# LeCAR-Lab/dial-mpc

Hardware: AMD Instinct MI355X
Metric: sample-rollouts/sec (N x H env.steps), Go2 N=2048 H=16 (higher is better)
Workload: dtype f32

## Files before the change

### dial_mpc_amd/csrc/rollout_body.h

```cpp
#pragma once
#include "derived.h"
#include "dmath.h"

#define MJ_MINVAL 1e-15f
#define MJ_MINIMP 0.0001f
#define MJ_MAXIMP 0.9999f
#define DIAL_PI 3.14159265358979323846f

namespace dial {

template <class D>
inline constexpr bool kNeedL = D::gen;

struct RowRef { int is_lim, dof, c, tan; float f; };
template <class M>
DIAL_DEV int con_of(const M*, const Ws& s, int c) {
  if constexpr (!M::D::gen) return c;
  else return (int)s.clist[c];
}
template <class M>
DIAL_DEV RowRef row_ref(const M* m, const Ws& s, int r) {
  RowRef rr;
  const int nl = dim_nl(m), nlf = nl + dim_nf(m);
  rr.is_lim = r < nlf;
// ... 923 lines not shown
    for (int k = 0; k < 3; k++) { fr[k] = n[k]; fr[3 + k] = bb[k]; fr[6 + k] = cc[k]; }
    float sgn = m->con_kind[c] == DIAL_CON_PLANE_CAPSULE_P ? 1.f : -1.f, hl = m->geom_size[g2][1];
    for (int k = 0; k < 3; k++) ctr[k] += sgn * axis[k] * hl;
  }
  float diff[3] = {ctr[0] - s.gpos[3 * g1], ctr[1] - s.gpos[3 * g1 + 1], ctr[2] - s.gpos[3 * g1 + 2]};
  float dist = dm::dot3(diff, n) - radius;
  s.cdist[c] = dist;
  for (int k = 0; k < 3; k++) s.cpos[3 * c + k] = ctr[k] - n[k] * (radius + 0.5f * dist);
  if constexpr (M::D::ell) s.con_on[c] = (dist - m->con_margin[c]) < 0.f ? 1.f : 0.f;
}

template <class W, class M>
DIAL_DEV void forward_tail(W& w, const M* m, const Ws& s) {
  const int nv = dim_nv(m), nc = dim_nc(m), ne = dim_ne(m), nl = dim_nl(m);
  int nca = nc, nea = ne;
  (void)nv; (void)nl;
  if constexpr (M::D::gen) {
    if (nc <= 64) {
      nca = w.compact(nc, [&](int c) { return s.cdist[c] - m->con_margin[c] < 0.f; }, s.clist);
    } else {
      w.items(nc, [&](int c) { s.clist[c] = (float)c; });
    }
    nea = nl + dim_nf(m) + 4 * nca;
  }
  if constexpr (M::D::gen) {
    if (s.con_cap > 0 && nca > s.con_cap && s.ovf != nullptr) {
      Ws sg = s;
      float* ovf = s.ovf;
#ifndef DIAL_EMU
      asm volatile("" : "+v"(ovf));
#endif
      ws_overflow(sg, ovf, nv, nc, ne);
      forward_constraints(w, m, sg, nca, nea);
      return;
    }
  }
  forward_constraints(w, m, s, nca, nea);
}

template <class W, class M>
DIAL_DEV void forward(W& w, const M* m, const Ws& s) {
  const int nb = dim_nb(m), nv = dim_nv(m), nj = dim_nj(m), ng = dim_ng(m), nsite = dim_ns(m), nc = dim_nc(m);
  const int ne = dim_ne(m), nl = dim_nl(m), ntri = m->ntri;
  int nca = nc, nea = ne;

  if constexpr (W::half2) {
    static_assert(kQuadDims<typename M::D>, "the half-wave kernel exists for the Go2's own instantiation");
    forward_smooth_quad2(w, m, s);
    forward_constraints(w, m, s, nca, nea);
    return;
  } else
  if constexpr (kQuadDims<typename M::D>) {
    forward_smooth_quad(w, m, s);
    forward_constraints(w, m, s, nca, nea);
    return;
  }
  if constexpr (kQuadGenDims<typename M::D>) {
    forward_smooth_quad<false>(w, m, s);
    w.items(nc, [&](int c) { collide_contact(m, s, c); });
    forward_tail(w, m, s);
    return;
  }
  if constexpr (kRowsGenDims<typename M::D>) {
    forward_smooth_rows<true>(w, m, s);
    w.items(nc, [&](int c) { collide_contact(m, s, c); });
    forward_tail(w, m, s);
    return;
  }
  if constexpr (kRowsDims<typename M::D>) {
    forward_smooth_rows(w, m, s);
    {
      DIAL_LANE_SCOPE_IF(DIAL_ROWS_PHASE_SCOPE, w);
      w.items(nc, [&](int c) { collide_contact(m, s, c); });
    }
    forward_constraints(w, m, s, nca, nea);
    return;
  }
  DIAL_MARK(w, 15);
  const bool kin_fast = m->kin_fast != 0;
  if (kin_fast) {
    vfloat L[9];
    w.per_lane_n(L, [&](int b, float* o) {
      for (int k = 0; k < 9; k++) o[k] = 0.f;
      o[7] = -1.f;
      if (b == 0 || b >= nb) return;
      const int bflags = m->body_flags[b];
      float lq[4] = {m->body_quat[b][0], m->body_quat[b][1], m->body_quat[b][2], m->body_quat[b][3]};
      float lp[3] = {m->body_pos[b][0], m->body_pos[b][1], m->body_pos[b][2]};
      if (m->body_jntnum[b] == 1) {
        const int ji = m->body_jntadr[b], qa = m->jnt_qposadr[ji], type = m->jnt_type[ji];
        const float jp[3] = {m->jnt_pos[ji][0], m->jnt_pos[ji][1], m->jnt_pos[ji][2]};
        const float ja[3] = {m->jnt_axis[ji][0], m->jnt_axis[ji][1], m->jnt_axis[ji][2]};
        if (type == DIAL_JNT_FREE) {
          for (int k = 0; k < 3; k++) lp[k] = s.qpos[qa + k];
          for (int k = 0; k < 4; k++) lq[k] = s.qpos[qa + 3 + k];
          dm::normalize4(lq);
          for (int k = 0; k < 4; k++) s.qpos[qa + 3 + k] = lq[k];
        } else if (type == DIAL_JNT_HINGE) {
          float qloc[4], qb[4], t0[3], t1[3];
          dm::axis_angle_to_quat(qloc, ja, s.qpos[qa] - m->qpos0[qa]);
          if (bflags & 1) { qb[0] = qloc[0]; qb[1] = qloc[1]; qb[2] = qloc[2]; qb[3] = qloc[3]; }
          else dm::quat_mul(qb, lq, qloc);
          if (!(bflags & 2)) {
            if (bflags & 1) { t0[0] = jp[0]; t0[1] = jp[1]; t0[2] = jp[2]; }
            else dm::rotate(t0, jp, lq);
            dm::rotate(t1, jp, qb);
// ... 572 lines not shown
  w.items(1 + nq, [&](int it) {
    if (it == 0) s.info[DIAL_INFO_STEP] += 1.f;
    else if (w.out_io && w.out_io->qss) w.out_io->qss[(size_t)w.out_row * nq + (it - 1)] = s.qpos[it - 1];
  });
}

template <bool EPI, class W>
DIAL_DEV int reward_items(const W& w, int n) {
  if constexpr (EPI) return w.epi_cnt;
  else return n;
}

template <bool FULL_INFO, bool PRE = false, bool EPI = false, class W, class M>
DIAL_DEV float env_step(W& w, const M* m, const dial_task* tg, const Ws& s, int st = 0) {
  const int nu = dim_nu(m);
  const bool walk = m->kind == DIAL_TASK_GO2_WALK || m->kind == DIAL_TASK_H1_WALK || m->kind == DIAL_TASK_H1_LOCO ||
                    m->kind == DIAL_TASK_H1_PUSH_CRATE;
  static_assert(!PRE || M::D::pre_ctrl, "control tables: carved for the Dims::pre_ctrl instantiations only");
  if constexpr (PRE) {
    w.jrow = s.jtab + st * nu;
  } else if constexpr (M::D::user_ctrl) {
    w.items(nu, [&](int a) {
      const bool tab = m->table_rows > 0;
      const DialControlIn in = control_in(m, s.info[DIAL_INFO_STEP], s.qpos, s.qvel, s.act, tab ? m->table_ring[m->table_half] : nullptr,
                                          tab ? m->table_cur : 0);
      const float c = dial_user_control(in, a, m->user_params, s.info + DIAL_INFO_USER);
      s.ctrl[a] = c;
      s.info[DIAL_INFO_LAST_CTRL + a] = c;
    });
  } else
  w.items(nu + DIAL_MAX_FEET, [&](int it) {
    if (it < nu) {
      const int a = it;
      const float jt = act2joint(m, s.act[a], a);
      float c;
      if (m->position_control) c = jt;
      else {
        float q_err = jt - s.qpos[7 + a];
        c = dm::clip(m->kp[a] * q_err - m->kd[a] * s.qvel[6 + a], m->tau_range[a][0], m->tau_range[a][1]);
      }
      s.ctrl[a] = c;
    } else {
      const int f = it - nu;
      if (walk && f < m->nfeet) s.ztar[f] = gait_ztar(m, f, s.info[DIAL_INFO_STEP]);
    }
  });
  DIAL_MARK(w, 25);
  const int n_frames = EPI ? 0 : (PRE ? 1 : m->n_frames);
  for (int f = 0; f < n_frames; f++) {
#ifndef DIAL_EMU
    if (w.launder) { asm volatile("" : "+v"(w.lane)); w.lane_r = w.lane; }
#endif
    forward(w, m, s);
    euler(w, m, s);
    DIAL_MARK(w, 9);
  }
  if constexpr (M::D::user) {
    w.items(1, [&](int) {
      float* info = s.info;
      const float step = info[DIAL_INFO_STEP];
      const bool tab = m->table_rows > 0;
      const DialRewardIn in{dim_nq(m), dim_nv(m), nu, dim_nb(m), dim_ns(m), dim_nc(m), step, m->dt,
                            s.qpos, s.qvel, s.xpos, s.xquat, s.spos, s.cdist, s.cpos, s.ctrl, s.act,
                            tab ? m->table_ring[m->table_half] : nullptr, tab ? m->table_cur : 0, m->table, m->table_rows, m->table_cols};
      const float reward = dial_user_reward(in, m->user_params, info + DIAL_INFO_USER);
      if (FULL_INFO) info[DIAL_INFO_DONE] = 0.f;
      info[DIAL_INFO_STEP] = step + 1.f;
      info[DIAL_INFO_REWARD] = reward;
    });
    DIAL_MARK(w, 10);
    return s.info[DIAL_INFO_REWARD];
  }
  if (m->kind == DIAL_TASK_ALLEGRO) {
    w.items(3, [&](int it) {
      const int ob = m->torso_x + 1;
      float acc = 0.f;
      if (it == 0) {
        for (int k = 0; k < 3; k++) { const float e = s.cvel[6 * ob + k] * DIAL_PI / 180.0f - s.info[DIAL_INFO_ANG_VEL_TAR + k]; acc += e * e; }
      } else if (it == 1) {
        for (int k = 0; k < 3; k++) { const float e = s.xpos[3 * ob + k] - s.info[DIAL_INFO_POS_TAR + k]; acc += e * e; }
      } else {
        for (int a = 0; a < nu; a++) { const float e = s.qpos[7 + a] - m->joint_offset[a]; acc += e * e; }
      }
      s.rpart[it] = acc;
    });
    w.items(1, [&](int) {
      const float step = s.info[DIAL_INFO_STEP];
      const float reward = -s.rpart[0] * 1.0f + -s.rpart[1] * 5.0f + -s.rpart[2] * 0.1f;
      if (FULL_INFO) s.info[DIAL_INFO_DONE] = step >= 100.f ? 1.f : 0.f;
      s.info[DIAL_INFO_STEP] = step + 1.f;
      s.info[DIAL_INFO_REWARD] = reward;
    });
    DIAL_MARK(w, 10);
    return s.info[DIAL_INFO_REWARD];
  }
  if constexpr (M::D::gen && ((task_kind_mask<typename M::D>() >> DIAL_TASK_GO2_CRATE) & 1u)) {
    if (m->kind == DIAL_TASK_GO2_CRATE) {
      w.items(1, [&](int) {
        float* info = s.info;
        const int tb = m->torso_x + 1, ub = m->upright_x + 1;
        const float step = info[DIAL_INFO_STEP], dt = m->dt;
        const float tq[4] = {s.xquat[4 * tb], s.xquat[4 * tb + 1], s.xquat[4 * tb + 2], s.xquat[4 * tb + 3]};
        const float uq[4] = {s.xquat[4 * ub], s.xquat[4 * ub + 1], s.xquat[4 * ub + 2], s.xquat[4 * ub + 3]};
        const float hv[3] = {m->head_vec[0], m->head_vec[1], m->head_vec[2]};
        float mat[9], head[3];
        dm::quat_to_mat(mat, tq);
// ... 305 lines not shown
```

### dial_mpc_amd/csrc/rollout_driver.h

```cpp
#pragma once
#include "rollout_body.h"
#include "philox.h"

namespace dial {


template <class W, class M>
DIAL_DEV void load_state(W& w, const M* m, const Ws& s, const float* state) {
  const int nq = dim_nq(m), nv = dim_nv(m);
  DIAL_LANE_SCOPE_IF(M::D::ell, w);
  w.items(nq + 2 * nv + DIAL_INFO_N, [&](int i) {
    float v = state[i];
    if (i < nq) s.qpos[i] = v;
    else if (i < nq + nv) s.qvel[i - nq] = v;
    else if (i < nq + 2 * nv) s.warm[i - nq - nv] = v;
    else s.info[i - nq - 2 * nv] = v;
  });
}
template <class W, class M>
DIAL_DEV void store_state(W& w, const M* m, const Ws& s, float* state) {
  const int nq = dim_nq(m), nv = dim_nv(m);
  DIAL_LANE_SCOPE_IF(M::D::ell, w);
  w.items(nq + 2 * nv + DIAL_INFO_N, [&](int i) {
    float v;
// ... 177 lines not shown
  };
  bool mean_now = false;
  constexpr int KSTRIDE = W::half2 ? 32 : 64, NKEEP = W::half2 ? 4 : 2;
  float keep[NKEEP] = {};
  rsum_t msum = 0;
  (void)packed; (void)keep; (void)msum;
  for (int st_own = st_begin; mean_now || st_own < st_end;) {
    const int st = mean_now ? helper : st_own;
    const int row = mean_now ? io.n_noise : n;
    w.redraw_priority();
#ifndef DIAL_EMU
    if (w.launder) { asm volatile("" : "+v"(w.lane)); w.lane_r = w.lane; }
    if constexpr (M::D::user) {
      if (trows > 0 && !mean_now) {
        const int idx = m->table_nidx, cols = m->table_cols;
        table_publish(w, m, st & 1, idx, cols, tnext);
        if (st + 1 < st_end) {
          M* const c = const_cast<M*>(m);
          const int r = m->table_nr + 1, nidx = table_next_index(idx, r, trows, m->table_mode);
          tnext = table_fetch(m, w.lane, nidx, cols);
          w.sync();
          if (w.lane == 0) { c->table_nidx = nidx; c->table_nr = r; }
        }
      }
    }
#endif
    if constexpr (!PRE) {
      DIAL_LANE_SCOPE_IF(kRowsDims<typename M::D> && !M::D::gen, w);
      w.items(nu, [&](int a) {
        float u;
        if (mean_now && !io.us) {
          u = 0.f;
          for (int k = 0; k < Hn1; k++) u += cfg->W[st][k] * dm::clip(io.Ybar[k * nu + a], -1.f, 1.f);
        } else {
          u = node2u(st, a);
        }
        s.act[a] = u;
      });
    } else {
#ifndef DIAL_EMU
      if (mean_now) {
        w.items(nu, [&](int a) {
          float u = 0.f;
          for (int k = 0; k < Hn1; k++) u += cfg->W[st][k] * dm::clip(io.Ybar[k * nu + a], -1.f, 1.f);
          s.jtab[st * nu + a] = act2joint(m, u, a);
        });
      }
#endif
    }
    DIAL_MARK(w, 11);
    const int work0 = w.work;
    if constexpr (PRE) { w.out_io = &io; w.out_row = row * T + st; }
    if constexpr (W::defer_rewards) reward_rows(w, st);
    float rew = env_step<false, PRE>(w, m, tg, s, st);
    if (mean_now) msum += (rsum_t)rew;
    else if constexpr (!W::defer_rewards) rsum += (rsum_t)rew;
#ifndef DIAL_EMU
    if constexpr (M::D::ell) {
      if (io.work_stat && relay < 0) {
        int lvl = 0;
        if (w.lane == 0) {
          const int tot_w = atomicAdd(io.work_stat, w.work - work0) + (w.work - work0);
          const int tot_s = atomicAdd(io.work_stat + 1, 1) + 1;
          const float own = (float)w.work * (float)tot_s, avg = (float)tot_w * (float)(st + 1 - st_begin);
#ifndef DIAL_LAG_T1
#define DIAL_LAG_T1 1.0f
#define DIAL_LAG_T2 1.2f
#define DIAL_LAG_T3 1.4f
#endif
          lvl = own > DIAL_LAG_T3 * avg ? 3 : (own > DIAL_LAG_T2 * avg ? 2 : (own > DIAL_LAG_T1 * avg ? 1 : 0));
        }
        w.prio_level = __builtin_amdgcn_readfirstlane(lvl);
      }
    }
#endif
    const size_t o = (size_t)row * T + st;
    if constexpr (!PRE) {
      float* const qrow = io.qss ? io.qss + o * nq : nullptr;
      float* const qdrow = io.qdss ? io.qdss + o * nv : nullptr;
      float* const xrow = io.xss ? io.xss + o * nx : nullptr;
      float* const rrow = io.rewss ? io.rewss + o : nullptr;
      const int nmax = nx > nq ? nx : nq;
      w.items(nmax, [&](int i) {
        if (qrow && i < nq) qrow[i] = s.qpos[i];
        if (qdrow && i < nv) qdrow[i] = s.qvel[i];
        if (xrow && i < nx) xrow[i] = s.xpos[3 + i];
        if (rrow && i == 0) rrow[0] = rew;
      });
    }
    (void)o;
#ifndef DIAL_PROFILE
    if constexpr (TRACE) { if (io.trace) store_state(w, m, s, io.trace + o * nstate); }
#endif
    DIAL_MARK(w, 24);
#ifndef DIAL_EMU
    if (mean_now) {
      if (helper + 1 < T) {
        store_state(w, m, s, io.relay_buf);
        w.items(1, [&](int) { store_sum(io.relay_buf + nstate, msum); });
        __builtin_amdgcn_fence(__ATOMIC_RELEASE, "agent");
        if (w.lane == 0) __hip_atomic_store(io.relay_flag, helper + 1, __ATOMIC_RELEASE, __HIP_MEMORY_SCOPE_AGENT);
      } else {
        if (io.rews) { const float mean = (float)(msum / (rsum_t)T); w.items(1, [&](int) { io.rews[row] = mean; }); }
        if (w.lane == 0) __hip_atomic_store(io.relay_flag, 0, __ATOMIC_RELEASE, __HIP_MEMORY_SCOPE_AGENT);
      }
      w.items(KSTRIDE, [&](int l) {
// ... 122 lines not shown
```

### dial_mpc_amd/csrc/solver_reg.h

```cpp
#pragma once

namespace dial {

template <int N> constexpr int kCholStride = (N + 3) & ~3;

template <class Topo, int N>
struct ElimOrder {
  int seq[N > 0 ? N : 1] = {};
  int nlevel = 0;
  int lvl[N > 0 ? N + 1 : 2] = {};
  constexpr ElimOrder() {
    int depth[N > 0 ? N : 1] = {};
    int maxd = 0;
    for (int i = 0; i < N; i++) {
      int d = 0;
      for (int j = 0; j < i; j++) d += Topo::anc(i, j) ? 1 : 0;
      depth[i] = d;
      maxd = d > maxd ? d : maxd;
    }
    int t = 0;
    for (int d = maxd; d >= 0; d--) {
      lvl[nlevel++] = t;
      for (int i = N - 1; i >= 0; i--)
        if (depth[i] == d) seq[t++] = N - 1 - i;
// ... 138 lines not shown
    w.dup_rows(b, bX, bY);
    static_for<l0, l1>([&](auto STEP) {
      constexpr int kp = EO.seq[STEP];
      const vfloat col = a[kp];
      vfloat cX, cY;
      w.dup_rows(col, cX, cY);
      const vfloat rinv = w.template rcp_pick<kp>(cX, cY);
      const vfloat lik = vsel(w.lane_gt(kp), col * rinv, vsplat(0.f));
      a[kp] = lik;
      dinv = vsel(w.lane_eq(kp), rinv, dinv);
      constexpr AncList<Topo, N, kp> L{};
      static_for<0, L.n>([&](auto IDX) {
        constexpr int jp = L.jp[IDX];
        a[jp] = w.template fnma_pick<jp>(a[jp], cX, cY, lik);
      });
    });
    static_for<l0, l1>([&](auto STEP) { constexpr int kp = EO.seq[STEP]; b = w.template fnma_pick<kp>(b, bX, bY, a[kp]); });
  });
  w.items(N, [&](int l) {
    static_for<0, N>([&](auto KP) { constexpr int kp = KP; scratch[(N - 1 - kp) * S + own_i(l)] = lane_val(a[kp], l); });
  });
  if (dinv_io) *dinv_io = dinv;
  }
  vfloat x = b * dinv;
  static_for<0, S / 4>([&](auto Q) {
    constexpr int q = Q;
    vfloat t[4];
    w.per_lane4([&](int l) { return scratch + (l < N ? own_i(l) : 0) * S + 4 * q; }, t[0], t[1], t[2], t[3]);
    static_for<0, 4>([&](auto E) {
      constexpr int j = 4 * q + E;
      if constexpr (j < N) a[N - 1 - j] = t[E];
    });
  });
  static_for<0, EO.nlevel>([&](auto LVR) {
    constexpr int lv = EO.nlevel - 1 - LVR, l0 = EO.lvl[lv], l1 = EO.lvl[lv + 1];
    vfloat xX, xY;
    w.dup_rows(x, xX, xY);
    static_for<l0, l1>([&](auto STEP) { constexpr int kp = EO.seq[STEP]; x = w.template fnma_pick<kp>(x, xX, xY, a[kp]); });
  });
  return w.lane_reverse(x, N);
}


#ifndef DIAL_CHOL_DPP
#define DIAL_CHOL_DPP 1
#endif
template <class D, class TopoT = typename D::Topo, bool REUSE = false, class W, class M>
DIAL_DEV vfloat reg_chol(W& w, const M* m, const float* A, vfloat bvec, float* scratch, vfloat* dinv_io = nullptr) {
  constexpr bool go2_one = std::is_same<D, DimsGo2>::value && !W::half2;
  if constexpr (W::half2 || (DIAL_CHOL_DPP && !go2_one)) return reg_chol_solve2<D, TopoT, REUSE>(w, m, A, bvec, scratch, dinv_io);
  else return reg_chol_solve_v<D, TopoT, REUSE>(w, m, A, bvec, scratch, dinv_io);
}

template <class W, class M>
DIAL_DEV void solver_reg(W& w, const M* m, const Ws& s) {
  constexpr int NV = M::D::NV, NC = M::D::NC, NL = M::D::NL;
  constexpr int C0 = 32;
  static_assert(NV <= 32 && 4 * NC <= 32, "lane layout needs nv <= 32 and 4*ncon <= 32");
  w.begin_region();
  const vbool isdof = w.lane_lt(NV);
  const vfloat vzero = vsplat(0.f);

  auto row_of = [&](int l) -> int {
    if (l < NV) return m->dof_limrow[l];
    if (l >= C0 && l < C0 + 4 * NC) return NL + (l - C0);
    return -1;
  };
  vfloat R[NV];
  {
    constexpr int S = M::D::S, T = M::D::T;
    const auto fetch = [&](int l, int j) {
      const int ojc = (int)(s.Jc - s.M), ozero = (int)(s.lsign - s.M) + NL;
      const int off = l < NV ? l * S : ((l >= C0 && l < C0 + 4 * NC) ? ojc + (l - C0) : ozero);
      const int stride = l < NV ? 1 : ((l >= C0 && l < C0 + 4 * NC) ? T : 0);
      return s.M[off + j * stride];
    };
#pragma unroll
    for (int j = 0; j < NV; j++) {
      if constexpr (NV > 20) R[j] = w.per_lane_r([&](int l) { return fetch(l, j); });
      else R[j] = w.per_lane([&](int l) { return fetch(l, j); });
    }
  }
  const vfloat vD = w.per_lane([&](int l) { int r = row_of(l); return r >= 0 ? s.D[r] : 0.f; });
  const vfloat varef = w.per_lane([&](int l) { int r = row_of(l); return r >= 0 ? s.aref[r] : 0.f; });
  const vfloat vls = w.per_lane([&](int l) { int r = l < NV ? m->dof_limrow[l] : -1; return r >= 0 ? s.lsign[r] : 0.f; });
  const vfloat vqfs = w.per_lane([&](int l) { return l < NV ? s.qfs[l] : 0.f; });
  const vfloat vqas = w.per_lane([&](int l) { return l < NV ? s.qas[l] : 0.f; });
  const vfloat vwarm = w.per_lane([&](int l) { return l < NV ? s.warm[l] : 0.f; });

#ifndef DIAL_SWEEP_DPP
#define DIAL_SWEEP_DPP 1
#endif
  auto dotR = [&](const vfloat& v) {
    vfloat acc[3] = {vzero, vzero, vzero};
#if DIAL_SWEEP_DPP
    vfloat vlo, vhi, X, Y;
    w.dup_halves(v, vlo, vhi);
    w.dup_rows(vlo, X, Y);
    static_for<0, NV>([&](auto IDX) { constexpr int j = IDX; acc[j % 3] = w.template fma_pick<j>(acc[j % 3], X, Y, R[j]); });
#else
    float sb[3] = {0.f, 0.f, 0.f};
    static_for<0, NV + 2>([&](auto IDX) {
      constexpr int idx = IDX;
      if constexpr (idx < NV) sb[idx % 3] = bcast(v, idx);
      if constexpr (idx >= 2) acc[(idx - 2) % 3] = acc[(idx - 2) % 3] + R[idx - 2] * sb[(idx - 2) % 3];
    });
#endif
    return (acc[0] + acc[1]) + acc[2];
  };
  auto row_prod = [&](const vfloat& v, const vfloat& sweep) { return vsel(isdof, vls * v, sweep); };
  auto row_cost_terms = [&](const vfloat& ja) { return vsel(vlt0(ja), vD * ja * ja, vzero); };

  const vfloat pW = dotR(vwarm), pS = dotR(vqas);
  const vfloat jaW = row_prod(vwarm, pW) - varef, jaS = row_prod(vqas, pS) - varef;
  const vfloat maW = vsel(isdof, pW, vzero), maS = vsel(isdof, pS, vzero);
  float cw, gw, cs, gs;
  {
    vfloat t[4] = {row_cost_terms(jaW), (maW - vqfs) * (vwarm - vqas), row_cost_terms(jaS), (maS - vqfs) * (vqas - vqas)};
    float r[4];
    w.vsumN(t, r);
    cw = r[0]; gw = r[1]; cs = r[2]; gs = r[3];
  }
  const float cost_w = 0.5f * cw + 0.5f * gw, cost_s = 0.5f * cs + 0.5f * gs;
  const bool use_warm = cost_w < cost_s;
  vfloat vqacc = use_warm ? vwarm : vqas;
  vfloat vMa = use_warm ? maW : maS;
  vfloat vJa = use_warm ? jaW : jaS;
  float cost = use_warm ? cost_w : cost_s;
  float gauss = use_warm ? 0.5f * gw : 0.5f * gs;
  float prev_cost = INFINITY;
  const float scale = 1.f / (m->meaninertia * (float)(NV > 1 ? NV : 1));
  const bool rule_swap = m->ls_rule == DIAL_LS_SWAP;
  const int max_iter = DM_UNIFORM_I(m->iterations), max_ls = DM_UNIFORM_I(m->ls_iterations);
  const float tol = m->tolerance, ls_tol = m->ls_tolerance, meaninertia = m->meaninertia;

#ifdef DIAL_PROFILE
  unsigned long long prof_prev_act = 0;
#endif
  int niter = 0;
  unsigned long long act_prev = 0;
  vfloat h_dinv = vzero;
  bool h_valid = false;
  for (;;) {
    const vbool act = vlt0(vJa);
#ifdef DIAL_PROFILE
    {
      const unsigned long long cur = __builtin_amdgcn_ballot_w64(act && (vD > 0.f));
      static_assert(sizeof(cur) == 8, "");
      if (niter == 1 && w.lane == 0 && w.acc) { w.acc[28] += 1; if (cur == prof_prev_act) w.acc[29] += 1; }
      prof_prev_act = cur;
    }
#endif
    const vfloat vf = vsel(act, vD * (vzero - vJa), vzero);
    vfloat qfc = vls * vf;
#if DIAL_SWEEP_DPP
    vfloat flo, fhi, fX, fY;
    w.dup_halves(vf, flo, fhi);
    w.dup_rows(fhi, fX, fY);
#endif
    static_for<0, NC>([&](auto Cc) {
      constexpr int c = Cc;
      vfloat jr[4];
      w.per_lane4([&](int l) { return s.Jc + (l < NV ? l : 0) * M::D::T + 4 * c; }, jr[0], jr[1], jr[2], jr[3]);
#if DIAL_SWEEP_DPP
      const vfloat t01 = w.template fma_pick<4 * c + 1>(w.template mul_pick<4 * c>(fX, fY, jr[0]), fX, fY, jr[1]);
      const vfloat t23 = w.template fma_pick<4 * c + 3>(w.template mul_pick<4 * c + 2>(fX, fY, jr[2]), fX, fY, jr[3]);
      qfc = qfc + (t01 + t23);
#else
      qfc = qfc + ((jr[0] * bcast(vf, C0 + 4 * c) + jr[1] * bcast(vf, C0 + 4 * c + 1)) +
                   (jr[2] * bcast(vf, C0 + 4 * c + 2) + jr[3] * bcast(vf, C0 + 4 * c + 3)));
#endif
    });
    const vfloat vgrad = vsel(isdof, vMa - vqfs - qfc, vzero);
    float gn = 0.f;
    if (niter > 0) {
      vfloat t[3] = {row_cost_terms(vJa), (vMa - vqfs) * (vqacc - vqas), vgrad * vgrad};
      float r[3];
      w.vsumN(t, r);
      gauss = 0.5f * r[1];
      prev_cost = cost;
      cost = 0.5f * r[0] + gauss;
      gn = r[2];
    } else if (max_iter != 1) {
      gn = w.vsum(vgrad * vgrad);
    }
    DIAL_MARK(w, 4);
    bool done;
    if (max_iter != 1) {
      const float improvement = scale * (prev_cost - cost), gradient = scale * DM_SQRT(gn);
      done = niter >= max_iter || improvement < tol || gradient < tol;
    } else {
      done = niter >= 1;
    }
    if (done) break;

    const vfloat vwgt = vsel(act, vD, vzero);
#ifdef DIAL_NO_FACTOR_REUSE
    const bool reuse = false;
#else
    const unsigned long long act_now = w.mask(vlt0(vzero - vwgt));
    const bool reuse = h_valid && act_now == act_prev;
    act_prev = act_now;
    h_valid = true;
#endif
    vfloat vsearch;
    if (reuse) {
      vsearch = vzero - reg_chol<typename M::D, typename M::D::Topo, true>(w, m, s.H, vgrad, s.H, &h_dinv);
      DIAL_MARK(w, 5);
    } else {
    {
      constexpr int S = M::D::S, T = M::D::T, NLP = M::D::NLP, NP = M::D::NHI / 64;
      (void)S;
      w.items(64, [&](int l) {
        const int r = row_of(l);
        if (r >= 0) s.frc[r < NL ? r : NLP + (r - NL)] = lane_val(vwgt, l);
        if (l == 63) s.frc[NLP + 4 * NC] = 0.f;
      });
      vfloat part[NP], tot[NP];
      static_for<0, 4>([&](auto Qq) {
        constexpr int q = Qq;
        bool any = false;
        static_for<0, NP>([&](auto PASS) { any = any || q < m->hpass_n[PASS]; });
        if (any) {
          vfloat ji[NP][4], jj[NP][4], dd[NP][4];
          static_for<0, NP>([&](auto PASS) {
            constexpr int pass = PASS;
            const auto c4 = [&](int l) { return (int)((m->hrec[pass * 64 + l][0] >> (20 + 3 * q)) & 7u) * 4; };
            w.per_lane4([&](int l) { return s.Jc + (m->hrec[pass * 64 + l][0] & 1023u) + c4(l); }, ji[pass][0], ji[pass][1], ji[pass][2], ji[pass][3]);
            w.per_lane4([&](int l) { return s.Jc + ((m->hrec[pass * 64 + l][0] >> 10) & 1023u) + c4(l); }, jj[pass][0], jj[pass][1], jj[pass][2], jj[pass][3]);
            w.per_lane4([&](int l) { return s.frc + NLP + c4(l); }, dd[pass][0], dd[pass][1], dd[pass][2], dd[pass][3]);
          });
          static_for<0, NP>([&](auto PASS) {
            constexpr int pass = PASS;
            const vfloat t = ((ji[pass][0] * dd[pass][0]) * jj[pass][0] + (ji[pass][1] * dd[pass][1]) * jj[pass][1]) +
                             ((ji[pass][2] * dd[pass][2]) * jj[pass][2] + (ji[pass][3] * dd[pass][3]) * jj[pass][3]);
            const vfloat tq = w.per_lane([&](int l) { return q < (int)(m->hrec[pass * 64 + l][1] >> 29) ? lane_val(t, l) : 0.f; });
            if constexpr (q == 0) part[pass] = tq; else part[pass] = part[pass] + tq;
          });
        }
      });
      static_for<0, NP>([&](auto PASS) {
        constexpr int pass = PASS;
        const vfloat pair = part[pass] + w.quad_xor1(part[pass]);
        const vfloat quad = pair + w.quad_xor2(pair);
        tot[pass] = w.per_lane([&](int l) {
          const float t1 = lane_val(part[pass], l), t2 = lane_val(pair, l), t4 = lane_val(quad, l);
          const uint32_t pc = (m->hrec[pass * 64 + l][1] >> 26) & 3u;
// ... 44 lines not shown
      ljv[q] = w.per_lane([&](int l) { const int r = (l & 15) + 16 * q; return (l < 48 && r < NE) ? s.jv[r] : 0.f; });
      const vfloat lD = w.per_lane([&](int l) { const int r = (l & 15) + 16 * q; return (l < 48 && r < NE) ? s.D[r] : 0.f; });
      const vfloat dja = lD * lJa[q], djv = lD * ljv[q];
      Q0[q] = (lJa[q] * 0.5f) * dja;
      Q1[q] = ljv[q] * dja;
      Q2[q] = (ljv[q] * 0.5f) * djv;
    }
    vfloat pk[4];
    auto ls_eval3 = [&](float a0, float a1, float a2) {
      const vfloat va = vsel(g0, vsplat(a0), vsel(g01, vsplat(a1), vsplat(a2)));
      vfloat s0 = vzero, s1v = vzero, s2v = vzero;
#pragma unroll
      for (int q = 0; q < RPL; q++) {
        const vfloat act = vsel(vlt0(lJa[q] + ljv[q] * va), vsplat(1.f), vzero);
        s0 = s0 + act * Q0[q];
        s1v = s1v + act * Q1[q];
        s2v = s2v + act * Q2[q];
      }
      w.row16_sum3(s0, s1v, s2v);
      const vfloat q0 = s0 + vsplat(qg0), q1 = s1v + vsplat(qg1), q2 = s2v + vsplat(qg2);
      const vfloat vcost = (va * va) * q2 + va * q1 + q0;
      const vfloat vd0 = vfma(va * 2.f, q2, q1);
      const vfloat vd1 = q2 * 2.f + vsel(veq0(q2), vsplat(MJ_MINVAL), vzero);
      w.per_lane_n(pk, [&](int l, float* o) {
        ls_pack(lane_val(va, l), lane_val(vcost, l), lane_val(vd0, l), lane_val(vd1, l), o[0], o[1], o[2], o[3]);
      });
    };
    auto point_at = [&](int lane) {
      LsPt p;
      p.alpha = fbits(bcast(pk[0], lane)); p.nalpha = fbits(bcast(pk[1], lane)); p.cost = fbits(bcast(pk[2], lane)); p.d0 = fbits(bcast(pk[3], lane));
      return p;
    };
    ls_eval3(0.f, 0.f, 0.f);
    const LsPt p0 = point_at(0);
    ls_eval3(bitsf(p0.nalpha), bitsf(p0.nalpha), bitsf(p0.nalpha));
    LsPt lo, hi;
    ls_open(p0, point_at(0), lo, hi);
    const int kg = DM_UNIFORM_I(fkey(gtol)), kng = DM_UNIFORM_I(fkey(-gtol));
    const LsGate gate = ls_gate(kg, kng);
    int ls_iter = 0;
    while (ls_iter < max_ls) {
      DM_NOFOLD();
      if (ls_converged_lo(lo, gate)) break;
      DM_NOFOLD();
      if (ls_converged_hi(hi, gate)) break;
      ls_eval3(bitsf(lo.nalpha), bitsf(hi.nalpha), 0.5f * (bitsf(lo.alpha) + bitsf(hi.alpha)));
      const bool swap = ls_update_lazy(rule_swap, lo, hi, fbits(bcast(pk[3], 0)), fbits(bcast(pk[3], 16)), fbits(bcast(pk[3], 32)), 0, 16, 32,
                                       [&](int word, int lane) { return fbits(bcast(pk[word], lane)); });
      ls_iter++;
      if (!swap) break;
    }
    float alpha;
    const bool improved = ls_result(p0, lo, hi, alpha);
    if (improved) {
      vqacc = vqacc + vsearch * alpha;
      vMa = vMa + vmv * alpha;
      vJa = vJa + vjv * alpha;
    }
    niter++;
#ifdef DIAL_PROFILE
    if (w.lane == 0 && w.acc) { w.acc[30] += ls_iter; w.acc[31] += 1; }
#endif
    DIAL_MARK(w, 7);
  }
  w.items(NV, [&](int i) {
    const float q = lane_val(vqacc, i);
    s.qacc[i] = q;
    s.warm[i] = q;
  });
  DIAL_MARK(w, 8);
}

}
```

### dial_mpc_amd/csrc/wave.h

```cpp
#pragma once
#include "rollout_io.h"

#ifdef DIAL_EMU
#include <cmath>
#include <cstdio>
#include <cstring>
#include <vector>
#define DIAL_DEV inline
#define DIAL_UNROLL


struct vbool { bool x[64]; };
struct vfloat {
  float x[64];
};
inline vfloat vsplat(float v) { vfloat r; for (int l = 0; l < 64; l++) r.x[l] = v; return r; }
inline vfloat operator+(const vfloat& a, const vfloat& b) { vfloat r; for (int l = 0; l < 64; l++) r.x[l] = a.x[l] + b.x[l]; return r; }
inline vfloat operator-(const vfloat& a, const vfloat& b) { vfloat r; for (int l = 0; l < 64; l++) r.x[l] = a.x[l] - b.x[l]; return r; }
inline vfloat operator*(const vfloat& a, const vfloat& b) { vfloat r; for (int l = 0; l < 64; l++) r.x[l] = a.x[l] * b.x[l]; return r; }
inline vfloat operator*(const vfloat& a, float b) { vfloat r; for (int l = 0; l < 64; l++) r.x[l] = a.x[l] * b; return r; }
inline vfloat vfma(const vfloat& a, const vfloat& b, const vfloat& c) { vfloat r; for (int l = 0; l < 64; l++) r.x[l] = std::fma(a.x[l], b.x[l], c.x[l]); return r; }
inline vfloat vsel(const vbool& c, const vfloat& a, const vfloat& b) { vfloat r; for (int l = 0; l < 64; l++) r.x[l] = c.x[l] ? a.x[l] : b.x[l]; return r; }
inline vbool vlt0(const vfloat& a) { vbool r; for (int l = 0; l < 64; l++) r.x[l] = a.x[l] < 0.f; return r; }
inline vbool veq0(const vfloat& a) { vbool r; for (int l = 0; l < 64; l++) r.x[l] = a.x[l] == 0.f; return r; }
inline float bcast(const vfloat& v, int lane) { return v.x[lane]; }
inline float lane_val(const vfloat& v, int lane) { return v.x[lane]; }
inline void load2(const float* p, float& a, float& b) { a = p[0]; b = p[1]; }
inline void load4(const float* p, float& a, float& b, float& c, float& d) { a = p[0]; b = p[1]; c = p[2]; d = p[3]; }
inline void store2(float* p, float a, float b) { p[0] = a; p[1] = b; }
inline void store4(float* p, float a, float b, float c, float d) { p[0] = a; p[1] = b; p[2] = c; p[3] = d; }
inline float fast_rsqrt(float x) { return 1.0f / std::sqrt(x); }
inline float fast_rcp(float x) { return 1.0f / x; }
inline vfloat vrcp(const vfloat& a) { vfloat r; for (int l = 0; l < 64; l++) r.x[l] = 1.0f / a.x[l]; return r; }

inline float emu_row_tree(const float* v) {
  float s1[16], s2[16], s3[16];
  for (int l = 0; l < 16; l++) s1[l] = v[l] + v[l ^ 1];
  for (int l = 0; l < 16; l++) s2[l] = s1[l] + s1[l ^ 2];
  for (int l = 0; l < 16; l++) s3[l] = s2[l] + s2[(l & 8) | (7 - (l & 7))];
  return s3[15] + s3[0];
}
inline float emu_tree64(const float* v) {
  const float r0 = emu_row_tree(v), r1 = emu_row_tree(v + 16), r2 = emu_row_tree(v + 32), r3 = emu_row_tree(v + 48);
  return (r3 + r2) + (r1 + r0);
}
inline float emu_tree32(const float* v) {
  return emu_row_tree(v) + emu_row_tree(v + 16);
}

#define DIAL_MARK(w, id)
#define DIAL_LANE_SCOPE(w)
#define DIAL_LANE_SCOPE_IF(cond, w)
struct Wave {
  static constexpr bool half2 = false;
  static constexpr bool defer_rewards = false;
  bool tree_sums = false;
  bool launder = false;
  const dial::RolloutIO* out_io = nullptr;
  int out_row = 0;
  const float* jrow = nullptr;
  float* lds = nullptr;
  int lds_words = 0;
  bool check_races = false;
  int races = 0;
  int phase = 0;

  bool nancheck = false, nan_seen = false;
  void scan_nonfinite() {
    if (!nancheck || nan_seen) return;
    for (int k = 0; k < lds_words; k++)
      if (!std::isfinite(lds[k])) {
        std::fprintf(stderr, "[wave_emu] first non-finite LDS word after phase #%d: word %d = %g\n", phase, k, (double)lds[k]);
        nan_seen = true;
        return;
      }
  }
  template <class F>
  void items(int count, F f) {
    phase++;
    if (!check_races) {
      for (int i = 0; i < count; i++) f(i);
      scan_nonfinite();
      return;
    }
    std::vector<float> snap(lds, lds + lds_words);
    for (int i = 0; i < count; i++) f(i);
    std::vector<float> fwd(lds, lds + lds_words);
    std::memcpy(lds, snap.data(), sizeof(float) * lds_words);
    for (int i = count - 1; i >= 0; i--) f(i);
    if (std::memcmp(fwd.data(), lds, sizeof(float) * lds_words) != 0) {
      if (races < 10) {
        int w = 0;
        for (; w < lds_words; w++)
          if (std::memcmp(&fwd[w], &lds[w], 4) != 0) break;
        std::fprintf(stderr, "[wave_emu] intra-phase dependence in phase #%d (first differing LDS word %d)\n", phase, w);
      }
      races++;
    }
  }
  template <class F>
  float sum(int count, F f) {
    if (tree_sums) {
      float v[64];
      for (int l = 0; l < 64; l++) { v[l] = l < count ? f(l) : 0.f; for (int i = l + 64; i < count; i += 64) v[l] += f(i); }
      return emu_tree64(v);
    }
    float s = 0.f;
    for (int i = 0; i < count; i++) s += f(i);
// ... 66 lines not shown
      float t = 0.f;
      for (int l = 0; l < 16; l++) t += v.x[16 * g + l];
      for (int l = 0; l < 16; l++) r.x[16 * g + l] = t;
    }
    return r;
  }
  void row16_sum3(vfloat& a, vfloat& b, vfloat& c) { a = row16_sum(a); b = row16_sum(b); c = row16_sum(c); }
  template <class F>
  int compact(int count, F pred, float* list) {
    int n = 0;
    for (int l = 0; l < count && l < 64; l++) if (pred(l)) list[n++] = (float)l;
    return n;
  }
  template <int K>
  void row16_sumN(vfloat (&v)[K]) { for (int k = 0; k < K; k++) v[k] = row16_sum(v[k]); }
  template <int K>
  void seg8_sumN(vfloat (&v)[K]) {
    for (int k = 0; k < K; k++) {
      vfloat s1, s2, s3;
      for (int l = 0; l < 64; l++) s1.x[l] = v[k].x[l] + v[k].x[l ^ 1];
      for (int l = 0; l < 64; l++) s2.x[l] = s1.x[l] + s1.x[l ^ 2];
      for (int l = 0; l < 64; l++) s3.x[l] = s2.x[l] + s2.x[(l & ~7) | (7 - (l & 7))];
      v[k] = s3;
    }
  }
  template <class F>
  vfloat gather64(const vfloat& v, F src) { vfloat r; for (int l = 0; l < 64; l++) r.x[l] = v.x[src(l) & 63]; return r; }
  float vsum(const vfloat& v) { if (tree_sums) return emu_tree64(v.x); float s = 0.f; for (int l = 0; l < 64; l++) s += v.x[l]; return s; }
  template <int K>
  void vsumN(vfloat (&v)[K], float (&out)[K]) { for (int k = 0; k < K; k++) out[k] = vsum(v[k]); }
  template <int K>
  float bc(const vfloat& v) { return v.x[K]; }
  void dup_rows(const vfloat& v, vfloat& X, vfloat& Y) {
    for (int l = 0; l < 64; l++) { X.x[l] = v.x[(l & 32) | (l & 15)]; Y.x[l] = v.x[(l & 32) | 16 | (l & 15)]; }
  }
  void dup_halves(const vfloat& v, vfloat& LO, vfloat& HI) {
    for (int l = 0; l < 64; l++) { LO.x[l] = v.x[l & 31]; HI.x[l] = v.x[32 | (l & 31)]; }
  }
  template <int K>
  float rowbc(const vfloat& v) { return v.x[K]; }
  template <int K>
  vfloat mul_pick(const vfloat& X, const vfloat& Y, const vfloat& other) { return other * pick<K>(X, Y); }
  template <int K>
  vfloat pick(const vfloat& X, const vfloat& Y) { if constexpr (K < 16) return row_bcast<K>(X); else return row_bcast<K - 16>(Y); }
  template <int K>
  vfloat fma_pick(const vfloat& acc, const vfloat& X, const vfloat& Y, const vfloat& other) { return acc + other * pick<K>(X, Y); }
  template <int K>
  vfloat fnma_pick(const vfloat& acc, const vfloat& X, const vfloat& Y, const vfloat& other) { return acc - other * pick<K>(X, Y); }
  template <int K>
  vfloat rcp_pick(const vfloat& X, const vfloat& Y) { return vrcp(pick<K>(X, Y)); }
};
struct WaveD : Wave {
  static constexpr bool defer_rewards = true;
  float* stash = nullptr;
  float* srow = nullptr;
  float* zrow = nullptr;
  float* zbase = nullptr;
  int epi_cnt = 0;
};

struct WaveH : Wave {
  static constexpr bool half2 = true;
  template <class F>
  float sum(int count, F f) {
    float v[32];
    for (int l = 0; l < 32; l++) { v[l] = l < count ? f(l) : 0.f; for (int i = l + 32; i < count; i += 32) v[l] += f(i); }
    return emu_tree32(v);
  }
  template <class F>
  void sum3(int count, F f, float& a, float& b, float& c) {
    float va[32], vb[32], vc[32];
    for (int l = 0; l < 32; l++) {
      va[l] = vb[l] = vc[l] = 0.f;
      if (l < count) f(l, va[l], vb[l], vc[l]);
      for (int i = l + 32; i < count; i += 32) { float x = 0.f, y = 0.f, z = 0.f; f(i, x, y, z); va[l] += x; vb[l] += y; vc[l] += z; }
    }
    a = emu_tree32(va); b = emu_tree32(vb); c = emu_tree32(vc);
  }
  template <class F>
  vfloat per_lane(F f) { vfloat r; for (int l = 0; l < 64; l++) r.x[l] = f(l & 31); return r; }
  template <class F>
  vfloat per_lane_r(F f) { return per_lane(f); }
  template <int K, class F>
  void per_lane_n(vfloat (&out)[K], F f) {
    for (int l = 0; l < 64; l++) { float o[K]; f(l & 31, o); for (int k = 0; k < K; k++) out[k].x[l] = o[k]; }
  }
  template <class F>
  void per_lane4(F f, vfloat& a, vfloat& b, vfloat& c, vfloat& d) {
    for (int l = 0; l < 64; l++) { const float* p = f(l & 31); a.x[l] = p[0]; b.x[l] = p[1]; c.x[l] = p[2]; d.x[l] = p[3]; }
  }
  unsigned long long mask(const vbool& c) const { unsigned long long b = 0; for (int l = 0; l < 32; l++) b |= (unsigned long long)(c.x[l] ? 1 : 0) << l; return b; }
  vbool lane_gt(int k) const { vbool r; for (int l = 0; l < 64; l++) r.x[l] = (l & 31) > k; return r; }
  vbool lane_eq(int k) const { vbool r; for (int l = 0; l < 64; l++) r.x[l] = (l & 31) == k; return r; }
  vbool lane_lt(int k) const { vbool r; for (int l = 0; l < 64; l++) r.x[l] = (l & 31) < k; return r; }
  vfloat lane_reverse(const vfloat& v, int n) { vfloat r; for (int l = 0; l < 64; l++) r.x[l] = (l & 31) < n ? v.x[(l & 32) + n - 1 - (l & 31)] : 0.f; return r; }
  float vsum(const vfloat& v) { return emu_tree32(v.x); }
  template <int K>
  void vsumN(vfloat (&v)[K], float (&out)[K]) { for (int k = 0; k < K; k++) out[k] = vsum(v[k]); }
  template <class F>
  vfloat gather(const vfloat& v, F src) { vfloat r; for (int l = 0; l < 64; l++) r.x[l] = v.x[(l & 32) | (src(l & 31) & 31)]; return r; }
  vfloat grp8_bcast3(const vfloat& v) { vfloat r; for (int l = 0; l < 64; l++) r.x[l] = v.x[(l & ~7) | 3]; return r; }
};

#else
#include <hip/hip_runtime.h>
#define DIAL_DEV __device__ __forceinline__
// ... 31 lines not shown

using vfloat = float;
using vbool = bool;
__device__ __forceinline__ vfloat vsplat(float v) { return v; }
__device__ __forceinline__ vfloat vfma(vfloat a, vfloat b, vfloat c) { return __builtin_fmaf(a, b, c); }
__device__ __forceinline__ vfloat vsel(vbool c, vfloat a, vfloat b) { return c ? a : b; }
__device__ __forceinline__ vbool vlt0(vfloat a) { return a < 0.f; }
__device__ __forceinline__ vbool veq0(vfloat a) { return a == 0.f; }
__device__ __forceinline__ float bcast(vfloat v, int lane) {
  return __builtin_bit_cast(float, __builtin_amdgcn_readlane(__builtin_bit_cast(int, v), lane));
}
__device__ __forceinline__ float lane_val(vfloat v, int) { return v; }
__device__ __forceinline__ void load2(const float* p, float& a, float& b) { const float2 t = *reinterpret_cast<const float2*>(p); a = t.x; b = t.y; }
__device__ __forceinline__ void load4(const float* p, float& a, float& b, float& c, float& d) { const float4 t = *reinterpret_cast<const float4*>(p); a = t.x; b = t.y; c = t.z; d = t.w; }
__device__ __forceinline__ void store2(float* p, float a, float b) { *reinterpret_cast<float2*>(p) = make_float2(a, b); }
__device__ __forceinline__ void store4(float* p, float a, float b, float c, float d) { *reinterpret_cast<float4*>(p) = make_float4(a, b, c, d); }
__device__ __forceinline__ float fast_rsqrt(float x) { return __builtin_amdgcn_rsqf(x); }
__device__ __forceinline__ float fast_rcp(float x) { return __builtin_amdgcn_rcpf(x); }
__device__ __forceinline__ vfloat vrcp(vfloat a) { return __builtin_amdgcn_rcpf(a); }

template <class W>
struct LaneScope {
  W& w;
  int keep, keep_r;
  __device__ __forceinline__ explicit LaneScope(W& w_) : w(w_), keep(w_.lane), keep_r(w_.lane_r) {
    int lq = w.lane;
    asm volatile("" : "+v"(lq));
    w.lane = lq;
    w.lane_r = lq;
  }
  __device__ __forceinline__ ~LaneScope() { w.lane = keep; w.lane_r = keep_r; }
};
#define DIAL_LANE_SCOPE(w) LaneScope<std::remove_reference_t<decltype(w)>> dial_lane_scope_(w)
template <bool COND, class W>
struct LaneScopeIf {
  __device__ __forceinline__ explicit LaneScopeIf(W&) {}
};
template <class W>
struct LaneScopeIf<true, W> : LaneScope<W> {
  __device__ __forceinline__ explicit LaneScopeIf(W& w_) : LaneScope<W>(w_) {}
};
#define DIAL_LANE_SCOPE_IF(cond, w) LaneScopeIf<(cond), std::remove_reference_t<decltype(w)>> dial_lane_scope_if_(w)
#ifdef DIAL_PROFILE
#define DIAL_NSEC 32
#define DIAL_MARK(w, id) (w).mark(id)
#elif defined(DIAL_ISA_MARKS)
#define DIAL_MARK(w, id) asm volatile("; DIAL_MARK %0" ::"n"(id))
#else
#define DIAL_MARK(w, id)
#endif
struct Wave {
  static constexpr bool half2 = false;
  static constexpr bool defer_rewards = false;
  int lane;
  const dial::RolloutIO* out_io = nullptr;
  int out_row = 0;
  const float* jrow = nullptr;
#ifdef DIAL_PROFILE
  unsigned long long tprev = 0;
  unsigned long long* acc = nullptr;
  __device__ __forceinline__ void mark(int id) {
    unsigned long long t = __builtin_readcyclecounter();
    if (lane == 0 && acc) acc[id] += t - tprev;
    tprev = t;
  }
#endif
  __device__ __forceinline__ void sync() {
#ifdef DIAL_BLOCK_SYNC
    __syncthreads();
#else
    __builtin_amdgcn_fence(__ATOMIC_RELEASE, "wavefront");
    __builtin_amdgcn_wave_barrier();
    __builtin_amdgcn_fence(__ATOMIC_ACQUIRE, "wavefront");
#endif
  }

  template <class F>
  __device__ __forceinline__ void items(int count, F f) {
    for (int i = lane; i < count; i += 64) f(i);
    sync();
  }
  template <class F>
  __device__ __forceinline__ float sum(int count, F f) {
    float v = lane < count ? f(lane) : 0.f;
    for (int i = lane + 64; i < count; i += 64) v += f(i);
    return dialwave::wave_sum(v);
  }
  template <class F>
  __device__ __forceinline__ void sum3(int count, F f, float& a, float& b, float& c) {
    float x = 0.f, y = 0.f, z = 0.f;
    if (lane < count) f(lane, x, y, z);
    for (int i = lane + 64; i < count; i += 64) {
      float x2 = 0.f, y2 = 0.f, z2 = 0.f;
      f(i, x2, y2, z2);
      x += x2; y += y2; z += z2;
    }
    vfloat t3[3] = {x, y, z};
    float r3[3];
    vsumN(t3, r3);
    a = r3[0]; b = r3[1]; c = r3[2];
  }
  template <class F>
  __device__ __forceinline__ float maxv(int count, F f) {
    float v = lane < count ? f(lane) : -INFINITY;
    for (int i = lane + 64; i < count; i += 64) { const float u = f(i); v = u > v ? u : v; }
    return dialwave::wave_max_shfl(v);
// ... 152 lines not shown
    Y = __builtin_bit_cast(float, r1);
#ifdef DIAL_FUSED_DPP
    asm("s_nop 1" : "+v"(X), "+v"(Y));
#endif
  }
  __device__ __forceinline__ void dup_halves(vfloat v, vfloat& LO, vfloat& HI) {
    const auto r = __builtin_amdgcn_permlane32_swap(__builtin_bit_cast(unsigned, v), __builtin_bit_cast(unsigned, v), false, false);
    const unsigned r0 = r[0], r1 = r[1];
    LO = __builtin_bit_cast(float, r0);
    HI = __builtin_bit_cast(float, r1);
  }
  template <int K>
  __device__ __forceinline__ float rowbc(vfloat v) { return row_bcast<K>(v); }
  template <int K>
  __device__ __forceinline__ vfloat pick(vfloat X, vfloat Y) { if constexpr (K < 16) return row_bcast<K>(X); else return row_bcast<K - 16>(Y); }
#ifdef DIAL_FUSED_DPP
#define DIAL_DPP_TAIL " row_newbcast:%3 row_mask:0xf bank_mask:0xf bound_ctrl:1"
  template <int K>
  __device__ __forceinline__ vfloat fma_pick(vfloat acc, vfloat X, vfloat Y, vfloat other) {
    asm("v_fmac_f32_dpp %0, %1, %2" DIAL_DPP_TAIL : "+v"(acc) : "v"(K < 16 ? X : Y), "v"(other), "n"(K & 15));
    return acc;
  }
  template <int K>
  __device__ __forceinline__ vfloat fnma_pick(vfloat acc, vfloat X, vfloat Y, vfloat other) {
    asm("v_fmac_f32_dpp %0, -%1, %2" DIAL_DPP_TAIL : "+v"(acc) : "v"(K < 16 ? X : Y), "v"(other), "n"(K & 15));
    return acc;
  }
  template <int K>
  __device__ __forceinline__ vfloat rcp_pick(vfloat X, vfloat Y) {
    vfloat r;
    asm("v_rcp_f32_dpp %0, %1 row_newbcast:%2 row_mask:0xf bank_mask:0xf bound_ctrl:1" : "=v"(r) : "v"(K < 16 ? X : Y), "n"(K & 15));
    return r;
  }
  template <int K>
  __device__ __forceinline__ vfloat mul_pick(vfloat X, vfloat Y, vfloat other) {
    vfloat r;
    asm("v_mul_f32_dpp %0, %1, %2" DIAL_DPP_TAIL : "=v"(r) : "v"(K < 16 ? X : Y), "v"(other), "n"(K & 15));
    return r;
  }
#undef DIAL_DPP_TAIL
#else
  template <int K>
  __device__ __forceinline__ vfloat mul_pick(vfloat X, vfloat Y, vfloat other) { return other * pick<K>(X, Y); }
  template <int K>
  __device__ __forceinline__ vfloat fma_pick(vfloat acc, vfloat X, vfloat Y, vfloat other) { return acc + other * pick<K>(X, Y); }
  template <int K>
  __device__ __forceinline__ vfloat fnma_pick(vfloat acc, vfloat X, vfloat Y, vfloat other) { return acc - other * pick<K>(X, Y); }
  template <int K>
  __device__ __forceinline__ vfloat rcp_pick(vfloat X, vfloat Y) { return vrcp(pick<K>(X, Y)); }
#endif
};
struct WaveD : Wave {
  static constexpr bool defer_rewards = true;
  float* stash = nullptr;
  float* srow = nullptr;
  float* zrow = nullptr;
  float* zbase = nullptr;
  int epi_cnt = 0;
};

struct WaveH : Wave {
  static constexpr bool half2 = true;
  int half;
  __device__ __forceinline__ void init(int tid) { lane = tid & 31; lane_r = lane; half = (tid >> 5) & 1; }
  template <class F>
  __device__ __forceinline__ void items(int count, F f) {
    for (int i = lane; i < count; i += 32) f(i);
    sync();
  }
  static __device__ __forceinline__ float half_combine(float v) {
    const auto r = __builtin_amdgcn_permlane16_swap(__builtin_bit_cast(unsigned, v), __builtin_bit_cast(unsigned, v), false, false);
    const unsigned r0 = r[0], r1 = r[1];
    return __builtin_bit_cast(float, r0) + __builtin_bit_cast(float, r1);
  }
  template <int K>
  __device__ __forceinline__ float bc(vfloat v) {
    static_assert(K >= 0 && K < 32, "logical lane");
    vfloat X, Y;
    dup_rows(v, X, Y);
    if constexpr (K < 16) return row_bcast<K>(X);
    else return row_bcast<K - 16>(Y);
  }
  template <class F>
  __device__ __forceinline__ vfloat gather(vfloat v, F src) { return __shfl(v, (src(lane) & 31) + 32 * half, 64); }
  __device__ __forceinline__ vfloat grp8_bcast3(vfloat v) {
    const vfloat a = row_bcast<3>(v), b = row_bcast<11>(v);
    return (lane & 8) ? b : a;
  }

  static __device__ __forceinline__ float opaque(float v) { asm("" : "+v"(v)); return v; }
  __device__ __forceinline__ vfloat row16_sum(vfloat v) { return Wave::row16_sum(opaque(v)); }
  template <int K>
  __device__ __forceinline__ void row16_sumN(vfloat (&v)[K]) {
#pragma unroll
    for (int k = 0; k < K; k++) v[k] = opaque(v[k]);
    Wave::row16_sumN(v);
  }
  __device__ __forceinline__ void row16_sum3(vfloat& a, vfloat& b, vfloat& c) { a = opaque(a); b = opaque(b); c = opaque(c); Wave::row16_sum3(a, b, c); }
  __device__ __forceinline__ float vsum(vfloat v) { return half_combine(row16_sum(v)); }
  template <int K>
  __device__ __forceinline__ void vsumN(vfloat (&v)[K], float (&out)[K]) {
    row16_sumN(v);
#pragma unroll
    for (int k = 0; k < K; k++) out[k] = half_combine(v[k]);
  }
  template <class F>
// ... 49 lines not shown
```

Baseline: 6.032 million.

## Skip dead final-step work and trim last solver iteration in deferred-reward waves

```diff
diff --git a/dial_mpc_amd/csrc/rollout_body.h b/dial_mpc_amd/csrc/rollout_body.h
--- a/dial_mpc_amd/csrc/rollout_body.h
+++ b/dial_mpc_amd/csrc/rollout_body.h
@@ -999,6 +999,7 @@
   } else
   if constexpr (kQuadDims<typename M::D>) {
     forward_smooth_quad(w, m, s);
+    if constexpr (W::lean_tail_cut) { if (w.tail_cut) return; }
     forward_constraints(w, m, s, nca, nea);
     return;
   }
@@ -1677,6 +1678,9 @@
     if (w.launder) { asm volatile("" : "+v"(w.lane)); w.lane_r = w.lane; }
 #endif
     forward(w, m, s);
+    if constexpr (W::lean_tail_cut) {
+      if (w.tail_cut) { DIAL_MARK(w, 9); return 0.f; }
+    }
     euler(w, m, s);
     DIAL_MARK(w, 9);
   }
diff --git a/dial_mpc_amd/csrc/rollout_driver.h b/dial_mpc_amd/csrc/rollout_driver.h
--- a/dial_mpc_amd/csrc/rollout_driver.h
+++ b/dial_mpc_amd/csrc/rollout_driver.h
@@ -253,6 +253,7 @@
     const int work0 = w.work;
     if constexpr (PRE) { w.out_io = &io; w.out_row = row * T + st; }
     if constexpr (W::defer_rewards) reward_rows(w, st);
+    if constexpr (W::lean_tail_cut) w.tail_cut = (st + 1 == T && !io.qss && !io.qdss && helper < 0 && !mean_now) ? 1 : 0;
     float rew = env_step<false, PRE>(w, m, tg, s, st);
     if (mean_now) msum += (rsum_t)rew;
     else if constexpr (!W::defer_rewards) rsum += (rsum_t)rew;
diff --git a/dial_mpc_amd/csrc/solver_reg.h b/dial_mpc_amd/csrc/solver_reg.h
--- a/dial_mpc_amd/csrc/solver_reg.h
+++ b/dial_mpc_amd/csrc/solver_reg.h
@@ -214,6 +214,9 @@
   else return reg_chol_solve_v<D, TopoT, REUSE>(w, m, A, bvec, scratch, dinv_io);
 }
 
+#ifndef DIAL_SOLVER_EXIT_HOOK
+#define DIAL_SOLVER_EXIT_HOOK(at_cap)
+#endif
 template <class W, class M>
 DIAL_DEV void solver_reg(W& w, const M* m, const Ws& s) {
   constexpr int NV = M::D::NV, NC = M::D::NC, NL = M::D::NL;
@@ -303,15 +306,18 @@
   unsigned long long act_prev = 0;
   vfloat h_dinv = vzero;
   bool h_valid = false;
+#ifdef DIAL_PROFILE
+  const auto prof_active_set = [&](const vfloat& ja) {
+    const unsigned long long cur = __builtin_amdgcn_ballot_w64(vlt0(ja) && (vD > 0.f));
+    static_assert(sizeof(cur) == 8, "");
+    if (niter == 1 && w.lane == 0 && w.acc) { w.acc[28] += 1; if (cur == prof_prev_act) w.acc[29] += 1; }
+    prof_prev_act = cur;
+  };
+#endif
   for (;;) {
     const vbool act = vlt0(vJa);
 #ifdef DIAL_PROFILE
-    {
-      const unsigned long long cur = __builtin_amdgcn_ballot_w64(act && (vD > 0.f));
-      static_assert(sizeof(cur) == 8, "");
-      if (niter == 1 && w.lane == 0 && w.acc) { w.acc[28] += 1; if (cur == prof_prev_act) w.acc[29] += 1; }
-      prof_prev_act = cur;
-    }
+    prof_active_set(vJa);
 #endif
     const vfloat vf = vsel(act, vD * (vzero - vJa), vzero);
     vfloat qfc = vls * vf;
@@ -354,7 +360,7 @@
     } else {
       done = niter >= 1;
     }
-    if (done) break;
+    if (done) { DIAL_SOLVER_EXIT_HOOK(niter > 0 && niter >= max_iter); break; }
 
     const vfloat vwgt = vsel(act, vD, vzero);
 #ifdef DIAL_NO_FACTOR_REUSE
@@ -505,16 +511,33 @@
     }
     float alpha;
     const bool improved = ls_result(p0, lo, hi, alpha);
-    if (improved) {
+    const auto end_pass = [&] {
+      niter++;
+#ifdef DIAL_PROFILE
+      if (w.lane == 0 && w.acc) { w.acc[30] += ls_iter; w.acc[31] += 1; }
+#endif
+      DIAL_MARK(w, 7);
+    };
+    if constexpr (W::solver_cap_exit) {
+      if (improved) vqacc = vqacc + vsearch * alpha;
+      if (niter + 1 >= max_iter) {
+        end_pass();
+#ifdef DIAL_PROFILE
+        prof_active_set(improved ? vJa + vjv * alpha : vJa);
+#endif
+        DIAL_SOLVER_EXIT_HOOK(true);
+        break;
+      }
+      if (improved) {
+        vMa = vMa + vmv * alpha;
+        vJa = vJa + vjv * alpha;
+      }
+    } else if (improved) {
       vqacc = vqacc + vsearch * alpha;
       vMa = vMa + vmv * alpha;
       vJa = vJa + vjv * alpha;
     }
-    niter++;
-#ifdef DIAL_PROFILE
-    if (w.lane == 0 && w.acc) { w.acc[30] += ls_iter; w.acc[31] += 1; }
-#endif
-    DIAL_MARK(w, 7);
+    end_pass();
   }
   w.items(NV, [&](int i) {
     const float q = lane_val(vqacc, i);
diff --git a/dial_mpc_amd/csrc/wave.h b/dial_mpc_amd/csrc/wave.h
--- a/dial_mpc_amd/csrc/wave.h
+++ b/dial_mpc_amd/csrc/wave.h
@@ -1,5 +1,12 @@
 #pragma once
 #include "rollout_io.h"
+
+#ifndef DIAL_DEFER_FULL_SOLVE
+#define DIAL_DEFER_FULL_SOLVE 0
+#endif
+#ifndef DIAL_DEFER_FULL_TAIL
+#define DIAL_DEFER_FULL_TAIL 0
+#endif
 
 #ifdef DIAL_EMU
 #include <cmath>
@@ -54,6 +61,7 @@
 struct Wave {
   static constexpr bool half2 = false;
   static constexpr bool defer_rewards = false;
+  static constexpr bool solver_cap_exit = false, lean_tail_cut = false;
   bool tree_sums = false;
   bool launder = false;
   const dial::RolloutIO* out_io = nullptr;
@@ -226,6 +234,8 @@
 };
 struct WaveD : Wave {
   static constexpr bool defer_rewards = true;
+  static constexpr bool solver_cap_exit = !DIAL_DEFER_FULL_SOLVE, lean_tail_cut = !DIAL_DEFER_FULL_TAIL;
+  int tail_cut = 0;
   float* stash = nullptr;
   float* srow = nullptr;
   float* zrow = nullptr;
@@ -363,6 +373,7 @@
 struct Wave {
   static constexpr bool half2 = false;
   static constexpr bool defer_rewards = false;
+  static constexpr bool solver_cap_exit = false, lean_tail_cut = false;
   int lane;
   const dial::RolloutIO* out_io = nullptr;
   int out_row = 0;
@@ -621,6 +632,8 @@
 };
 struct WaveD : Wave {
   static constexpr bool defer_rewards = true;
+  static constexpr bool solver_cap_exit = !DIAL_DEFER_FULL_SOLVE, lean_tail_cut = !DIAL_DEFER_FULL_TAIL;
+  int tail_cut = 0;
   float* stash = nullptr;
   float* srow = nullptr;
   float* zrow = nullptr;
```

Result: faster. 6.117 million (median of 6 runs) (+1.4%).
